# batra-mlp-lab/visdial

Measured on NVIDIA H100. Metric: QA-rounds/sec mn-att-ques-im-hist+disc train step, higher is better.
Workload: dtype f16 operands + f16 saved state for the option LSTM, tf32 operands elsewhere; fp32 accumulate, fp32 cell state / gradients / optimiser

## Files before the change

### visdial_b200/csrc/engine.cu

```cuda
#include "engine.h"
#include <string.h>
#include <math.h>
#include <cmath>

namespace vd {

Cfg parse_cfg(const vd_params* p) {
  VD_REQUIRE(p && p->encoder && p->decoder, VD_E_BADARG, "params / encoder / decoder is null");
  Cfg c;
  c.encoder = p->encoder; c.decoder = p->decoder;
  struct { const char* name; int enc; } known[] = {
      {"lf-ques", ENC_LF_QUES}, {"lf-ques-im-hist", ENC_LF_QIH}, {"hrea-ques-im-hist", ENC_HREA}, {"mn-att-ques-im-hist", ENC_MN_ATT},
      {"lf-ques-im", ENC_LF_QI}, {"lf-ques-hist", ENC_LF_QH}, {"hre-ques-hist", ENC_HRE_QH}, {"hre-ques-im-hist", ENC_HRE_QIH},
      {"mn-ques-hist", ENC_MN_QH}, {"mn-ques-im-hist", ENC_MN_QIH}, {"lf-att-ques-im-hist", ENC_LF_ATT}};
  c.enc = -1;
  for (auto& k : known)
    if (c.encoder == k.name) c.enc = k.enc;
  VD_REQUIRE(c.enc >= 0, VD_E_BADARG, "unknown encoder (one of the eleven names of encoders/*.lua)");
  if (c.decoder == "disc") c.dec = DEC_DISC;
  else if (c.decoder == "gen") c.dec = DEC_GEN;
  else VD_REQUIRE(false, VD_E_BADARG, "unknown decoder (disc | gen)");
  c.V = p->vocabSize; c.E = p->embedSize; c.H = p->rnnHiddenSize; c.L = p->numLayers; c.F = p->imgFeatureSize;
  c.S = p->imgSpatialSize; c.IE = p->imgEmbedSize; c.Cm = p->commonEmbeddingSize; c.hops = p->numAttentionLayers;
  c.R = p->maxQuesCount; c.K = p->numOptions; c.dropout = p->dropout; c.gpuid = p->gpuid;
// ... 53 lines not shown
    }
    add_linear(l, "san.out", c.H, c.H);
  };
  if (c.fam_lf && !c.san) {
    add_lstm(l, "ques.lstm1", c.E, c.H); add_lstm(l, "ques.lstm2", c.H, c.H);
    if (c.useHist) { add_lstm(l, "hist.lstm1", c.E, c.H); add_lstm(l, "hist.lstm2", c.H, c.H); }
    add_linear(l, "fusion", c.H, c.H + (c.useIm ? c.F : 0) + (c.useHist ? c.H : 0));
  } else if (c.fam_hre) {
    if (c.img_in_q) add_linear(l, "img.embed", c.IE, c.F);
    add_lstm(l, "hist.lstm1", c.E, c.H); add_lstm(l, "hist.lstm2", c.H, c.H);
    add_lstm(l, "ques.lstm1", c.E + (c.img_in_q ? c.IE : 0), c.H); add_lstm(l, "ques.lstm2", c.H, c.H);
    if (c.hre_att) { add_linear(l, "att.q", 1, c.H); add_linear(l, "att.h", 1, c.H); }
    add_lstm(l, "dialog.lstm", 2 * c.H, c.H);
  } else {
    add_lstm(l, "hist.lstm1", c.E, c.H); add_lstm(l, "hist.lstm2", c.H, c.H);
    add_lstm(l, "ques.lstm1", c.E, c.H); add_lstm(l, "ques.lstm2", c.H, c.H);
    if (c.fam_lf) add_linear(l, "fusion", c.H, 2 * c.H);
    if (c.mn_qi) add_linear(l, "mn.qi", c.H, c.H + c.F);
    if (c.fam_mn) { add_linear(l, "mn.fact", c.H, c.H); add_linear(l, "mn.query", c.H, c.H); }
    if (c.san) add_san();
  }
  if (c.dec == DEC_DISC) {
    add_lstm(l, "opt.lstm", c.E, c.H);
  } else {
    add_lstm(l, "dec.lstm1", c.E, c.H); add_lstm(l, "dec.lstm2", c.H, c.H);
    add_linear(l, "dec.out", c.V, c.H);
  }
  return l;
}

void* Arena::alloc(size_t bytes) {
  bytes = (bytes + 255) & ~(size_t)255;
  if (bytes == 0) bytes = 256;
  while (cur < chunks.size()) {
    Chunk& c = chunks[cur];
    if (c.used + bytes <= c.cap) { void* p = c.p + c.used; c.used += bytes; return p; }
    ++cur;
  }
  Chunk c; c.cap = std::max<size_t>(bytes, (size_t)256 << 20); c.used = bytes;
  VD_CUDA_CHECK(cudaMalloc((void**)&c.p, c.cap));
  chunks.push_back(c);
  cur = chunks.size() - 1;
  return c.p;
}
void Arena::reset() { for (auto& c : chunks) c.used = 0; cur = 0; }
void Arena::release() { for (auto& c : chunks) cudaFree(c.p); chunks.clear(); cur = 0; }
void Arena::rewind(const Mark& m) {
  for (size_t i = m.chunk; i < chunks.size(); ++i) chunks[i].used = i == m.chunk ? m.used : 0;
  cur = m.chunk;
}

void* GrowBuf::ensure(size_t bytes) {
  if (bytes > cap) {
    if (p) cudaFree(p);
    p = nullptr; cap = 0;
    VD_CUDA_CHECK(cudaMalloc(&p, bytes));
    cap = bytes;
  }
  return p;
}
void GrowBuf::release() { if (p) cudaFree(p); p = nullptr; cap = 0; }

Engine::Engine(const vd_params* p) {
  cfg = parse_cfg(p);
  lay = build_layout(cfg);
  nparams = lay.total;
  int ndev = 0;
  VD_CUDA_CHECK(cudaGetDeviceCount(&ndev));
  VD_REQUIRE(cfg.gpuid >= 0 && cfg.gpuid < ndev, VD_E_BADARG, "gpuid out of range");
  VD_CUDA_CHECK(cudaSetDevice(cfg.gpuid));
  cudaDeviceProp prop;
  VD_CUDA_CHECK(cudaGetDeviceProperties(&prop, cfg.gpuid));
  VD_REQUIRE(prop.major == 9 && prop.minor == 0, VD_E_CUDA, "visdial_b200 is built for sm_90a (H100) only");
  cx.sm_count = prop.multiProcessorCount;
  int prio_lo = 0, prio_hi = 0;
  VD_CUDA_CHECK(cudaDeviceGetStreamPriorityRange(&prio_lo, &prio_hi));
  VD_CUDA_CHECK(cudaStreamCreateWithPriority(&cx.stream, cudaStreamNonBlocking, prio_hi));
  main_stream = cx.stream;
  VD_CUDA_CHECK(cudaStreamCreateWithPriority(&side_stream, cudaStreamNonBlocking, prio_hi));
  main_chain.a = main_stream; side_chain.a = side_stream;
  for (cudaStream_t* s : {&main_chain.b, &side_chain.b, &main_chain.c, &side_chain.c})
    VD_CUDA_CHECK(cudaStreamCreateWithPriority(s, cudaStreamNonBlocking, prio_hi));
  VD_CUDA_CHECK(cudaStreamCreateWithPriority(&opt_stream, cudaStreamNonBlocking, prio_lo));
  VD_CUDA_CHECK(cudaEventCreateWithFlags(&ev_fork, cudaEventDisableTiming));
  VD_CUDA_CHECK(cudaEventCreateWithFlags(&ev_join, cudaEventDisableTiming));
  VD_CUDA_CHECK(cudaEventCreateWithFlags(&ev_opt_fork, cudaEventDisableTiming));
  VD_CUDA_CHECK(cudaEventCreateWithFlags(&ev_opt_done, cudaEventDisableTiming));
  size_t bytes = (size_t)nparams * sizeof(float);
  VD_CUDA_CHECK(cudaMalloc((void**)&W, bytes));
  VD_CUDA_CHECK(cudaMalloc((void**)&dW, bytes));
  VD_CUDA_CHECK(cudaMalloc((void**)&m, bytes));
  VD_CUDA_CHECK(cudaMalloc((void**)&v, bytes));
  VD_CUDA_CHECK(cudaMalloc((void**)&Wt, bytes));
  VD_CUDA_CHECK(cudaMemsetAsync(W, 0, bytes, cx.stream));
  VD_CUDA_CHECK(cudaMemsetAsync(dW, 0, bytes, cx.stream));
  VD_CUDA_CHECK(cudaMemsetAsync(m, 0, bytes, cx.stream));
  VD_CUDA_CHECK(cudaMemsetAsync(v, 0, bytes, cx.stream));
  VD_CUDA_CHECK(cudaMemsetAsync(Wt, 0, bytes, cx.stream));
  VD_CUDA_CHECK(cudaMalloc((void**)&scalars_dev, 64 * sizeof(float)));
  std::vector<int64_t> tab;
  for (auto& s : lay.segs) {
    if (s.init == VD_INIT_LSTM_W || s.init == VD_INIT_LINEAR_W) {
      tab.push_back(s.off); tab.push_back(s.rows); tab.push_back(s.cols);
      max2d = std::max(max2d, s.rows * s.cols);
    }
  }
  nseg2d = (int)tab.size() / 3;
  VD_CUDA_CHECK(cudaMalloc((void**)&segtab_dev, tab.size() * sizeof(int64_t)));
  VD_CUDA_CHECK(cudaMemcpyAsync(segtab_dev, tab.data(), tab.size() * sizeof(int64_t), cudaMemcpyHostToDevice, cx.stream));
  VD_CUDA_CHECK(cudaStreamSynchronize(cx.stream));
  VD_CUDA_CHECK(cudaEventCreate(&t0));
  VD_CUDA_CHECK(cudaEventCreate(&t1));
}

Engine::~Engine() {
  cudaSetDevice(cfg.gpuid);
  cudaStreamSynchronize(cx.stream);
  if (opt_stream) cudaStreamSynchronize(opt_stream);
  arena.release();
  for (auto& g : stage) g.release();
  for (auto& g : dense_buf) g.release();
  dialog_hist.release();
  for (auto& g : dialog_out) g.release();
  if (copy_stream) {
    cudaStreamSynchronize(copy_stream); cudaStreamDestroy(copy_stream);
    cudaEventDestroy(ev_img_ready); cudaEventDestroy(ev_copy_fork);
    for (auto ev : ev_img_free) cudaEventDestroy(ev);
  }
  for (auto& g : stage_img) g.release();
  cudaFree(W); cudaFree(dW); cudaFree(m); cudaFree(v); cudaFree(Wt); cudaFree(scalars_dev); cudaFree(segtab_dev);
  if (flush_buf) cudaFree(flush_buf);
  cx.collect();
  for (auto e : cx.free_events) cudaEventDestroy(e);
  if (t0) cudaEventDestroy(t0);
  if (t1) cudaEventDestroy(t1);
  if (ev_fork) cudaEventDestroy(ev_fork);
  if (ev_join) cudaEventDestroy(ev_join);
  if (side_stream) { cudaStreamSynchronize(side_stream); cudaStreamDestroy(side_stream); }
  for (cudaStream_t s : {main_chain.b, side_chain.b, main_chain.c, side_chain.c})
    if (s) { cudaStreamSynchronize(s); cudaStreamDestroy(s); }
  if (opt_stream) { cudaStreamSynchronize(opt_stream); cudaStreamDestroy(opt_stream); }
  if (ev_opt_fork) cudaEventDestroy(ev_opt_fork);
  if (ev_opt_done) cudaEventDestroy(ev_opt_done);
  for (auto e : ev_pool) cudaEventDestroy(e);
  cudaStreamDestroy(main_stream);
}

int Engine::seg(const char* name) const {
  int i = lay.find(name);
  VD_REQUIRE(i >= 0, VD_E_STATE, name);
  return i;
}

DropCfg Engine::dropcfg(float p) const {
  DropCfg d;
  d.seed_lo = (uint32_t)drop_seed; d.seed_hi = (uint32_t)(drop_seed >> 32); d.iter = (uint32_t)drop_iter;
  if (training == 1 && p > 0.f) {
    double t = (double)p * 4294967296.0;
    d.thresh = (uint32_t)std::min(t, 4294967295.0);
    d.scale = 1.f / (1.f - p);
  } else { d.thresh = 0; d.scale = 1.f; }
  return d;
}

void Engine::gemm_tn(int M, int N, int K, const float* A, int64_t lda, const int32_t* gather, const float* B, int64_t ldb,
                     float* C, int64_t ldc, float beta, const float* bias, int act) {
  LaunchCtx::Scope sc(&cx, "gemm", 2.0 * M * N * K, 4.0 * ((double)M * K + (double)N * K + (double)M * N));
  if (tcmode() && gemm_tn_tc(cx, M, N, K, A, lda, gather, B, ldb, C, ldc, beta, bias, act)) return;
  gemm_tn_simt(cx, M, N, K, A, lda, gather, B, ldb, C, ldc, beta, bias, act);
}
void Engine::gemm_atb(int M, int N, int64_t K, const float* A, int64_t lda, const int32_t* gather, const float* B,
                      int64_t ldb, float* C, int64_t ldc) {
  LaunchCtx::Scope sc(&cx, "gemm_wgrad", 2.0 * M * N * K, 4.0 * ((double)M * K + (double)N * K + (double)M * N));
  if (tcmode() && gemm_atb_tc(cx, M, N, K, A, lda, gather, B, ldb, C, ldc)) return;
  gemm_atb_simt(cx, M, N, K, A, lda, gather, B, ldb, C, ldc);
}

void Engine::linear_fwd(int wseg, const float* x, int64_t rows, float* y, int act) {
  const Seg& s = lay.segs[wseg];
  gemm_tn((int)rows, (int)s.rows, (int)s.cols, x, s.cols, nullptr, Wp(wseg), s.cols, y, s.rows, 0.f, Wp(wseg + 1), act);
}
void Engine::linear_bwd(int wseg, const float* x, const float* dy, int64_t rows, float* dx, float beta_dx) {
  const Seg& s = lay.segs[wseg];
  int out = (int)s.rows, in = (int)s.cols;
  gemm_atb(out, in, rows, dy, out, nullptr, x, in, dWp(wseg), in);
  colsum_add(cx, dWp(wseg + 1), dy, rows, out, out);
  if (dx) gemm_tn((int)rows, in, out, dy, out, nullptr, Wtp(wseg), out, dx, in, beta_dx, nullptr, 0);
}

void Engine::refresh_shadows() {
  VD_CUDA_CHECK(cudaMemsetAsync(W, 0, (size_t)cfg.E * sizeof(float), cx.stream));
  transpose_segments(cx, W, Wt, segtab_dev, nseg2d, max2d);
}

void Engine::stage_batch(const vd_batch* b) {
  VD_REQUIRE(b != nullptr, VD_E_BADARG, "batch is null");
  VD_REQUIRE(b->B > 0, VD_E_SHAPE, "batch B must be > 0");
  db = DevBatch();
  db.B = b->B; db.N = (int64_t)b->B * cfg.R;
  db.Tq = b->Tq; db.Th = b->Th; db.Ta = b->Ta; db.To = b->To;
  VD_REQUIRE(b->ques_fwd && b->Tq > 0, VD_E_SHAPE, "ques_fwd / Tq missing");
  if (cfg.useHist) VD_REQUIRE(b->hist && b->Th > 0, VD_E_SHAPE, "encoder uses history: hist / Th missing");
  if (cfg.useIm) VD_REQUIRE(b->img_feat, VD_E_SHAPE, "encoder uses the image: img_feat missing");
  int64_t img_elems = cfg.att ? (int64_t)b->B * cfg.S * cfg.S * cfg.F : (int64_t)b->B * cfg.F;
  struct Item { const void* src; size_t bytes; const void** dst; } items[9] = {
      {b->ques_fwd, (size_t)db.N * b->Tq * 4, (const void**)&db.ques},
      {cfg.useHist ? b->hist : nullptr, (size_t)db.N * b->Th * 4, (const void**)&db.hist},
      {cfg.useIm ? b->img_feat : nullptr, (size_t)img_elems * 4, (const void**)&db.img},
      {b->options, (size_t)db.N * cfg.K * b->To * 4, (const void**)&db.options},
      {b->answer_ind, (size_t)db.N * 4, (const void**)&db.answer_ind},
      {b->answer_in, (size_t)db.N * b->Ta * 4, (const void**)&db.answer_in},
      {b->answer_out, (size_t)db.N * b->Ta * 4, (const void**)&db.answer_out},
      {b->option_in, (size_t)db.N * cfg.K * b->To * 4, (const void**)&db.option_in},
      {b->option_out, (size_t)db.N * cfg.K * b->To * 4, (const void**)&db.option_out}};
  img_copy_pending = false;
  for (int i = 0; i < 9; ++i) {
    if (!items[i].src || items[i].bytes == 0) { *items[i].dst = nullptr; continue; }
    if (b->on_device) { *items[i].dst = items[i].src; continue; }
    if (i == 2 && items[i].bytes >= ((size_t)1 << 20)) {
      if (!copy_stream) {
        VD_CUDA_CHECK(cudaStreamCreateWithFlags(&copy_stream, cudaStreamNonBlocking));
        VD_CUDA_CHECK(cudaEventCreateWithFlags(&ev_img_ready, cudaEventDisableTiming));
        VD_CUDA_CHECK(cudaEventCreateWithFlags(&ev_copy_fork, cudaEventDisableTiming));
        for (int k = 0; k < 2; ++k) VD_CUDA_CHECK(cudaEventCreateWithFlags(&ev_img_free[k], cudaEventDisableTiming));
      }
      img_slot ^= 1;
// ... 232 lines not shown
    VD_CUDA_CHECK(cudaEventRecord(ex, s.c));
    VD_CUDA_CHECK(cudaStreamWaitEvent(s.b, ex, 0));
    cx.stream = s.b;
    lstm_forward_step(l2, t, true);
  }
  VD_CUDA_CHECK(cudaEventRecord(e0, s.b));
  VD_CUDA_CHECK(cudaStreamWaitEvent(s.a, e0, 0));
  cx.stream = s.a;
}

void Engine::lstm_backward_begin(LstmRun& r, const float* dh_all, const float* dh_last, const float* dc_last) {
  VD_REQUIRE(r.saved, VD_E_STATE, "lstm_backward needs a forward run in training mode");
  const int H = r.H, G = 4 * r.H;
  const int64_t R = r.R, TR = (int64_t)r.T * R;
  r.dc_carry = arena.get<float>(R * H);
  r.bw_dh_all = dh_all; r.bw_dh_last = dh_last;
  if (r.route.bwd == LstmPath::Opt16) {
    VD_REQUIRE(dh_last && !dh_all && !dc_last, VD_E_STATE, "fp16 BPTT takes its gradient from the last step only");
    r.da16 = arena.get<__half>(TR * G);
    r.scale2 = arena.get<float>(4);
    pick_grad_scale(cx, dh_last, R * H, reinterpret_cast<uint32_t*>(r.scale2 + 2), r.scale2);
    return;
  }
  r.da = arena.get<float>(TR * G);
  r.dh_rec = arena.get<float>(R * H);
  if (dc_last)
    VD_CUDA_CHECK(cudaMemcpyAsync(r.dc_carry, dc_last, (size_t)R * H * sizeof(float), cudaMemcpyDeviceToDevice, cx.stream));
  else
    VD_CUDA_CHECK(cudaMemsetAsync(r.dc_carry, 0, (size_t)R * H * sizeof(float), cx.stream));
}

void Engine::lstm_backward_step(LstmRun& r, int t) {
  const int H = r.H, G = 4 * r.H;
  const int64_t R = r.R, RH = R * H, RG = R * G;
  const bool last = t == r.T - 1;
  const float* cp = t > 0 ? r.c + (t - 1) * RH : r.c0;
  const int32_t* mk = r.mask ? r.mask + (int64_t)t * R : nullptr;
  if (r.route.bwd == LstmPath::Opt16) {
    const __half* g16 = r.gates16 + t * RG;
    __half* da16_t = r.da16 + t * RG;
    if (last) {
      LaunchCtx::Scope sc(&cx, "lstm_step_bwd_last", 0.0, R * (2.0 * G + 2.0 * G + 16.0 * H));
      lstm16_bwd_last(cx, R, H, g16, cp, r.c + t * RH, r.bw_dh_last, r.scale2, mk, r.dc_carry, da16_t);
    } else {
      LaunchCtx::Scope sc(&cx, "lstm_step_bwd", 2.0 * R * G * H, R * (3.0 * 2.0 * G + 16.0 * H));
      lstm16_step_bwd(cx, R, H, r.da16 + (t + 1) * RG, r.Whb16, g16, cp, r.c + t * RH, r.dc_carry, mk, da16_t);
    }
    return;
  }
  LstmBwdStep s;
  s.R = R; s.H = H; s.Wh = Wp(r.wseg) + (int64_t)r.D * G; s.dc_carry = r.dc_carry; s.dh_rec = r.dh_rec; s.mask = mk;
  s.da_next = last ? nullptr : r.da + (t + 1) * RG; s.dh_last = last ? r.bw_dh_last : nullptr;
  s.dh_ext = r.bw_dh_all ? r.bw_dh_all + t * RH : nullptr;
  s.gates = r.gates + t * RG; s.c_prev = cp; s.c_cur = r.c + t * RH; s.da = r.da + t * RG;
  const bool tc = r.route.bwd == LstmPath::Tc;
  LaunchCtx::Scope sc(&cx, (last && tc) ? "lstm_step_bwd_last" : (R >= 4096 ? "lstm_step_bwd" : "lstm_step_bwd_small"),
                      last ? 0.0 : 2.0 * R * G * H, 4.0 * R * (2.0 * G + 5.0 * H));
  if (tc) lstm_tc_bwd_step(s); else lstm_simt_bwd_step(s);
}

void Engine::lstm_backward_end(LstmRun& r, float* dx_out, float* dh0_out, float* dc0_out) {
  const int H = r.H, D = r.D, G = 4 * r.H;
  const int64_t R = r.R, TR = (int64_t)r.T * R;
  const float* Ws = Wp(r.wseg);
  float* dWs = dWp(r.wseg);
  const bool opt16 = r.route.bwd == LstmPath::Opt16;
  if (opt16) VD_REQUIRE(!dh0_out && !dc0_out && !dx_out && !r.h0, VD_E_STATE, "fp16 BPTT: no initial-state / input gradients");
  if (dh0_out) gemm_tn((int)R, H, G, r.da, G, nullptr, Ws + (int64_t)D * G, G, dh0_out, H, 0.f, nullptr, 0);
  if (dc0_out) VD_CUDA_CHECK(cudaMemcpyAsync(dc0_out, r.dc_carry, (size_t)R * H * sizeof(float), cudaMemcpyDeviceToDevice, cx.stream));
  const bool wgrad16 = opt16 || (r.route.bwd == LstmPath::Pair16 && TR - R >= 256);
  if (r.T > 1) {
    if (wgrad16) {
      LaunchCtx::Scope sc(&cx, "gemm_wgrad", 2.0 * H * G * (double)(TR - R), 2.0 * (double)(TR - R) * (H + G));
      const int budget = cx.sm_budget;
      cx.sm_budget = 0;
      gemm_atb16(cx, H, G, TR - R, r.h16, H, r.da16 + R * G, G, dWs + (int64_t)D * G, G, r.scale2 + 1);
      cx.sm_budget = budget;
    } else gemm_atb(H, G, TR - R, r.h, H, nullptr, r.da + R * G, G, dWs + (int64_t)D * G, G);
  }
  if (r.h0) gemm_atb(H, G, R, r.h0, H, nullptr, r.da, G, dWs + (int64_t)D * G, G);
  if (r.route.table_grad) {
    VD_REQUIRE(dx_out == nullptr, VD_E_STATE, "projected-space embedding gradient: caller must not ask for dx");
    const int V1 = cfg.V + 1;
    float* dP = arena.get<float>((int64_t)V1 * G);
    VD_CUDA_CHECK(cudaMemsetAsync(dP, 0, (size_t)V1 * G * sizeof(float), cx.stream));
    int32_t* scratch = arena.get<int32_t>(3 * (int64_t)V1);
    int32_t* perm = arena.get<int32_t>(TR);
    int32_t* stok = arena.get<int32_t>(TR);
    {
      LaunchCtx::Scope sc(&cx, "embed_grad_segsum", 0.0, (opt16 ? 2.0 : 4.0) * TR * G);
      group_rows_by_token(cx, r.gather, TR, V1, scratch, perm, stok);
      if (opt16) segsum_rows16(cx, r.da16, G, perm, stok, TR, dP, G, r.scale2 + 1);
      else segsum_rows(cx, r.da, G, perm, stok, TR, dP, G);
    }
    gemm_atb(D, G, V1, Wp(0), cfg.E, nullptr, dP, G, dWs, G);
    colsum_add(cx, dWp(r.wseg + 1), dP, V1, G, G);
    if (r.demb_out) gemm_tn(V1, D, G, dP, G, nullptr, Ws, G, r.demb_out, cfg.E, 0.f, nullptr, 0);
    else gemm_tn(V1, D, G, dP, G, nullptr, Ws, G, dWp(0), cfg.E, 1.f, nullptr, 0);
    return;
  }
  if (wgrad16 && r.x16) {
    LaunchCtx::Scope sc(&cx, "gemm_wgrad", 2.0 * D * G * (double)TR, 2.0 * (double)TR * (D + G));
    gemm_atb16(cx, D, G, TR, r.x16, D, r.da16, G, dWs, G, r.scale2 + 1);
  } else gemm_atb(D, G, TR, r.x ? r.x : Wp(0), r.x ? D : cfg.E, r.gather, r.da, G, dWs, G);
  colsum_add(cx, dWp(r.wseg + 1), r.da, TR, G, G);
  if (dx_out) gemm_tn((int)TR, D, G, r.da, G, nullptr, Ws, G, dx_out, D, 0.f, nullptr, 0);
}

void Engine::lstm_backward(LstmRun& r, const float* dh_all, const float* dh_last, const float* dc_last, float* dx_out,
                           float* dh0_out, float* dc0_out) {
  lstm_backward_begin(r, dh_all, dh_last, dc_last);
  for (int t = r.T - 1; t >= 0; --t) lstm_backward_step(r, t);
  lstm_backward_end(r, dx_out, dh0_out, dc0_out);
}

void Engine::lstm_pair_backward(LstmRun& l1, LstmRun& l2, const float* dh_last2, const float* dc_last2, const float* dh_last1,
                                const float* dc_last1, float* dx1_out, const PairStreams& s) {
  const int H = l2.H, G = 4 * l2.H;
  const int64_t R = l2.R;
  cx.stream = s.a;
  if (l1.route.bwd == LstmPath::Pair16) {
    const int T = l2.T;
    const int64_t TR = (int64_t)T * R;
    l1.da = arena.get<float>(TR * G); l2.da = arena.get<float>(TR * G);
    l1.da16 = arena.get<__half>(TR * G); l2.da16 = arena.get<__half>(TR * G);
    __half* Whb2 = arena.get<__half>((int64_t)H * G);
    __half* B1cat = arena.get<__half>((int64_t)H * 2 * G);
    cvt_f32_to_f16(cx, Whb2, G, Wp(l2.wseg) + (int64_t)l2.D * G, G, H, G);
    cvt_f32_to_f16(cx, B1cat, 2 * G, Wp(l2.wseg), G, H, G);
    cvt_f32_to_f16(cx, B1cat + G, 2 * G, Wp(l1.wseg) + (int64_t)l1.D * G, G, H, G);
    int* flags = arena.get<int>(enc_pair_bwd_flag_ints(T, R, H));
    float* dh1 = nullptr; float* dh2 = nullptr;
    if (enc_pair_gate_split(H)) { dh1 = arena.get<float>(TR * H); dh2 = arena.get<float>(TR * H); }
    l1.scale2 = l2.scale2 = arena.get<float>(2);
    {
      LaunchCtx::Scope sc2(&cx, "enc_pair_bwd", 2.0 * T * R * (double)H * 3.0 * G, 4.0 * T * R * (4.0 * G + 4.0 * H));
      enc_pair_backward(cx, T, R, H, B1cat, Whb2, l1.mask, l1.gates, l1.c, l2.gates, l2.c, dh_last1, dc_last1, dh_last2, dc_last2,
                        l1.da, l1.da16, l2.da, l2.da16, flags, dh1, dh2, l1.scale2);
    }
    lstm_backward_end(l2, nullptr, nullptr, nullptr);
    lstm_backward_end(l1, dx1_out, nullptr, nullptr);
    return;
  }
  float* dx2 = arena.get<float>((int64_t)l2.T * R * l2.D);
  if (!l1.route.wave_bwd) {
    lstm_backward(l2, nullptr, dh_last2, dc_last2, dx2, nullptr, nullptr);
    lstm_backward(l1, dx2, dh_last1, dc_last1, dx1_out, nullptr, nullptr);
    return;
  }
  const float* Wx2 = Wp(l2.wseg);
  cudaEvent_t e0 = pool_event(0);
  VD_CUDA_CHECK(cudaEventRecord(e0, s.a));
  VD_CUDA_CHECK(cudaStreamWaitEvent(s.b, e0, 0));
  cx.stream = s.b;
  lstm_backward_begin(l2, nullptr, dh_last2, dc_last2);
  cx.stream = s.a;
  lstm_backward_begin(l1, dx2, dh_last1, dc_last1);
  for (int t = l2.T - 1; t >= 0; --t) {
    cx.stream = s.b;
    lstm_backward_step(l2, t);
    cudaEvent_t e = pool_event(1 + t);
    VD_CUDA_CHECK(cudaEventRecord(e, s.b));
    VD_CUDA_CHECK(cudaStreamWaitEvent(s.c, e, 0));
    cx.stream = s.c;
    gemm_tn((int)R, l2.D, G, l2.da + (int64_t)t * R * G, G, nullptr, Wx2, G, dx2 + (int64_t)t * R * l2.D, l2.D, 0.f, nullptr, 0);
    cudaEvent_t ex = pool_event(1 + l2.T + t);
    VD_CUDA_CHECK(cudaEventRecord(ex, s.c));
    VD_CUDA_CHECK(cudaStreamWaitEvent(s.a, ex, 0));
    cx.stream = s.a;
    lstm_backward_step(l1, t);
  }
  cx.stream = s.b;
  lstm_backward_end(l2, nullptr, nullptr, nullptr);
  VD_CUDA_CHECK(cudaEventRecord(e0, s.b));
  cx.stream = s.a;
  lstm_backward_end(l1, dx1_out, nullptr, nullptr);
  VD_CUDA_CHECK(cudaStreamWaitEvent(s.a, e0, 0));
}

static LstmRun make_run(int T, int64_t R, int D, int H, int wseg, const float* x, const int32_t* gather, const int32_t* mask) {
  LstmRun r; r.T = T; r.R = R; r.D = D; r.H = H; r.wseg = wseg; r.x = x; r.gather = gather; r.mask = mask;
  return r;
}

void Engine::mn_block_fwd(const float* qin, const float* h3, float* out) {
  const int H = cfg.H, R = cfg.R, B = db.B;
  const int64_t N = db.N;
  const DropCfg d05 = dropcfg(0.5f);
  probs = arena.get<float>((int64_t)B * R * R);
// ... 276 lines not shown
      san_block_bwd(dEnc, du);
      mn_block_bwd(du, qh2, dqin, dh3);
    } else {
      mn_block_bwd(dEnc, encOut, dqin, dh3);
    }
    if (cfg.mn_qi) {
      tanh_bwd(cx, dpre, dqin, qi_proj, N * H);
      float* dqj = arena.get<float>(N * (H + cfg.F));
      linear_bwd(seg("mn.qi.weight"), qi_join, dpre, N, dqj, 0.f);
      copy_cols(cx, dq3, H, dqj, H + cfg.F, N, H);
    }
    if (cfg.san) reduce_segments(seg(cfg.mn_qi ? "mn.qi.weight" : "mn.fact.weight"), seg("san.out.weight") + 1, main_stream);
  }

  const bool embdrop = cfg.embdrop;
  if (cfg.useHist) {
    if (serial_pairs()) join_side(); else fork_side();
    const PairStreams& hs = serial_pairs() ? main_chain : side_chain;
    float* dx1 = arena.get<float>(N * db.Th * E);
    lstm_pair_backward(hist1, hist2, dh3, nullptr, nullptr, nullptr, dx1, hs);
    reduce_segments(seg("hist.lstm1.weight"), seg("hist.lstm2.weight") + 1, hs.a);
    embed_scatter_add(cx, dWp(0), dx1, E, ids_h, N * db.Th, E, embdrop ? d05 : dnone, SITE_HEMBED);
    back_to_main();
  }
  {
    int D1 = ques1.D;
    float* dx1 = arena.get<float>(N * db.Tq * D1);
    lstm_pair_backward(ques1, ques2, dq3, conn_dc_l2, conn_dh_l1, conn_dc_l1, dx1, main_chain);
    reduce_segments(seg("ques.lstm1.weight"), seg("ques.lstm2.weight") + 1, main_stream);
    embed_scatter_add(cx, dWp(0), dx1, D1, ids_q, N * db.Tq, E, embdrop ? d05 : dnone, SITE_QEMBED);
    if (cfg.img_in_q) {
      float* die = arena.get<float>(N * cfg.IE);
      masktime_bwd(cx, dx1, D1, E, ids_q, die, db.Tq, N, cfg.IE);
      linear_bwd(seg("img.embed.weight"), img_d, die, N, nullptr, 0.f);
    }
  }
  join_side();
  join_options_backward();
}

void Engine::fork_side() {
  if (!side_active) {
    VD_CUDA_CHECK(cudaEventRecord(ev_fork, main_stream));
    VD_CUDA_CHECK(cudaStreamWaitEvent(side_stream, ev_fork, 0));
    side_active = true;
  }
  cx.stream = side_stream;
}
void Engine::back_to_main() { cx.stream = main_stream; }
void Engine::join_side() {
  cx.stream = main_stream;
  if (side_active) {
    VD_CUDA_CHECK(cudaEventRecord(ev_join, side_stream));
    VD_CUDA_CHECK(cudaStreamWaitEvent(main_stream, ev_join, 0));
    side_active = false;
  }
}

void Engine::forward_connect() {
  if (cfg.dec != DEC_GEN) return;
  VD_REQUIRE(have_fwd, VD_E_STATE, "forward_connect before encoder_forward");
  gen_h0[0] = gen_h0[1] = gen_c0[0] = gen_c0[1] = nullptr;
  if (cfg.rnn_layers) {
    gen_h0[0] = ques1.h_last(); gen_c0[0] = ques1.c_last();
    gen_c0[1] = ques2.c_last();
  }
  gen_h0[1] = encOut;
}

void Engine::options_forward_async() {
  const int64_t Ro = (dense_round ? db.B : db.N) * cfg.K;
  cudaStream_t s = opt_overlap ? opt_stream : main_stream;
  if (opt_overlap) {
    VD_CUDA_CHECK(cudaEventRecord(ev_opt_fork, main_stream));
    VD_CUDA_CHECK(cudaStreamWaitEvent(opt_stream, ev_opt_fork, 0));
  }
  cudaStream_t prev = cx.stream;
  cx.stream = s;
  if (opt_overlap) cx.sm_budget = cx.sm_count - (math_mode == VD_MATH_F16 ? 0 : opt_reserve_sms);
  ids_o = arena.get<int32_t>(Ro * db.To);
  if (dense_round) transpose_ids_rounds(cx, db.options, dense_round, ids_o, db.B, cfg.R, cfg.K, db.To);
  else transpose_ids(cx, db.options, ids_o, Ro, db.To);
  opt = make_run(db.To, Ro, cfg.E, cfg.H, seg("opt.lstm.weight"), nullptr, ids_o, nullptr);
  lstm_forward(opt, save_acts);
  VD_CUDA_CHECK(cudaEventRecord(ev_opt_done, s));
  cx.stream = prev;
  cx.sm_budget = 0;
  opt_fwd_pending = true;
}

void Engine::join_options_backward() {
  if (!opt_bwd_pending) return;
  opt_bwd_pending = false;
  cudaStream_t prev = cx.stream;
  cx.stream = main_stream;
  VD_CUDA_CHECK(cudaStreamWaitEvent(main_stream, ev_opt_done, 0));
  if (opt_demb) add_inplace(cx, dWp(0), opt_demb, (int64_t)(cfg.V + 1) * cfg.E);
  opt_demb = nullptr;
  cx.stream = prev;
}

void Engine::decoder_forward() {
  VD_REQUIRE(have_fwd, VD_E_STATE, "decoder_forward before encoder_forward");
  const int E = cfg.E, H = cfg.H, K = cfg.K;
  const int64_t N = db.N;
  if (cfg.dec == DEC_DISC) {
    VD_REQUIRE(db.options && db.To > 0, VD_E_SHAPE, "disc decoder: options / To missing");
    if (!opt_fwd_pending) options_forward_async();
    VD_CUDA_CHECK(cudaStreamWaitEvent(main_stream, ev_opt_done, 0));
    opt_fwd_pending = false;
    cx.stream = main_stream;
    scores = arena.get<float>(N * K);
    disc_scores_fwd(cx, opt.h_last(), encOut, scores, N, K, H);
  } else {
    VD_REQUIRE(db.answer_in && db.Ta > 0, VD_E_SHAPE, "gen decoder: answer_in / Ta missing");
    forward_connect();
    ids_ai = arena.get<int32_t>(N * db.Ta);
    transpose_ids(cx, db.answer_in, ids_ai, N, db.Ta);
    float* xa = arena.get<float>(N * db.Ta * E);
    embed_rows(cx, xa, Wp(0), ids_ai, N * db.Ta, E, dropcfg(0.f), 0);
    dec1 = make_run(db.Ta, N, E, H, seg("dec.lstm1.weight"), xa, nullptr, ids_ai);
    dec1.h0 = gen_h0[0]; dec1.c0 = gen_c0[0];
    lstm_forward(dec1, true);
    dec2 = make_run(db.Ta, N, H, H, seg("dec.lstm2.weight"), dec1.h, nullptr, ids_ai);
    dec2.h0 = gen_h0[1]; dec2.c0 = gen_c0[1];
    lstm_forward(dec2, true);
    fused_vocab_fwd = false;
    const int64_t rows = N * db.Ta;
    const int wo = seg("dec.out.weight");
    if (!want_logp && tcmode() && db.answer_out) {
      ids_ao = arena.get<int32_t>(rows);
      transpose_ids(cx, db.answer_out, ids_ao, N, db.Ta);
      voc_nparts = vocab_lse_nparts(cfg.V);
      voc_pm = arena.get<float>(rows * voc_nparts); voc_ps = arena.get<float>(rows * voc_nparts);
      voc_tl = arena.get<float>(rows); voc_lse = arena.get<float>(rows);
      LaunchCtx::Scope sc(&cx, "vocab_lse", 2.0 * rows * cfg.V * H, 4.0 * (rows * (double)H + (double)cfg.V * H + 2.0 * rows * voc_nparts));
      fused_vocab_fwd = vocab_lse_tc(cx, (int)rows, cfg.V, H, dec2.h, H, Wp(wo), H, Wp(wo + 1), ids_ao, voc_pm, voc_ps, voc_tl);
    }
    if (!fused_vocab_fwd) {
      logp = arena.get<float>(rows * cfg.V);
      linear_fwd(wo, dec2.h, rows, logp, 0);
      logsoftmax_rows(cx, logp, ids_ai, rows, cfg.V);
    } else {
      logp = nullptr;
    }
  }
}

float Engine::criterion_forward() {
  const int64_t N = db.N;
  if (cfg.dec == DEC_DISC) {
    VD_REQUIRE(scores && db.answer_ind, VD_E_STATE, "criterion: decoder_forward / answer_ind missing");
    row_loss = arena.get<float>(N);
    xent_fwd(cx, scores, db.answer_ind, row_loss, N, cfg.K);
    reduce_sum(cx, row_loss, scalars_dev, N, 1.f / (float)N);
  } else {
    VD_REQUIRE((logp || fused_vocab_fwd) && db.answer_out, VD_E_STATE, "criterion: decoder_forward / answer_out missing");
    row_loss = arena.get<float>(N * db.Ta);
    if (fused_vocab_fwd) {
      vocab_lse_finish(cx, voc_pm, voc_ps, voc_nparts, voc_tl, ids_ao, ids_ai, voc_lse, row_loss, -1.f, 0, N * db.Ta);
    } else {
      ids_ao = arena.get<int32_t>(N * db.Ta);
      transpose_ids(cx, db.answer_out, ids_ao, N, db.Ta);
      nll_fwd(cx, logp, ids_ao, ids_ai, row_loss, N * db.Ta, cfg.V);
    }
    reduce_sum(cx, row_loss, scalars_dev, N * db.Ta, 1.f);
  }
// ... 597 lines not shown
```

### visdial_b200/csrc/engine.h

```cpp
#pragma once
#include <functional>
#include <string>
#include <vector>
#include "../../include/visdial_b200.h"
#include "kernels.cuh"

namespace vd {

enum EncKind { ENC_LF_QUES = 0, ENC_LF_QIH = 1, ENC_HREA = 2, ENC_MN_ATT = 3, ENC_LF_QI = 4, ENC_LF_QH = 5, ENC_HRE_QH = 6, ENC_HRE_QIH = 7,
               ENC_MN_QH = 8, ENC_MN_QIH = 9, ENC_LF_ATT = 10 };
enum DecKind { DEC_DISC = 0, DEC_GEN = 1 };

struct Cfg {
  std::string encoder, decoder;
  int enc = 0, dec = 0;
  int V = 0, E = 300, H = 512, L = 2, F = 4096, S = 14, IE = 300, Cm = 512, hops = 1, R = 10, K = 100;
  float dropout = 0.5f;
  int gpuid = 0;
  bool useIm = false, useHist = false, att = false;
  bool fam_lf = false, fam_hre = false, fam_mn = false;
  bool hre_att = false;
  bool san = false;
  bool img_in_q = false;
  bool img_drop = false;
  bool mn_qi = false;
  bool embdrop = false;
  bool rnn_layers = false;
};
Cfg parse_cfg(const vd_params* p);

struct Seg {
  std::string name;
  int64_t off = 0, rows = 0, cols = 0;
  int init = 0;
  int64_t fan_in = 0;
};
struct Layout {
  std::vector<Seg> segs;
  int64_t total = 0;
  int find(const std::string& name) const;
};
Layout build_layout(const Cfg& c);

struct Arena {
  struct Chunk { char* p; size_t cap; size_t used; };
  std::vector<Chunk> chunks;
  size_t cur = 0;
  void* alloc(size_t bytes);
  template <typename T> T* get(int64_t n) { return reinterpret_cast<T*>(alloc((size_t)n * sizeof(T))); }
  void reset();
  void release();
  struct Mark { size_t chunk, used; };
  Mark mark() const { return {cur, cur < chunks.size() ? chunks[cur].used : 0}; }
  void rewind(const Mark& m);
};

enum class LstmPath { Simt, Tc, Opt16, Pair16 };
struct LstmRoute {
  LstmPath fwd = LstmPath::Simt, bwd = LstmPath::Simt;
  bool table_grad = false;
  bool wave_fwd = false, wave_bwd = false;
};

struct LstmRun {
  int T = 0; int64_t R = 0; int D = 0, H = 0;
  int wseg = -1;
  const float* x = nullptr;
  const int32_t* gather = nullptr;
  const int32_t* mask = nullptr;
  const float* h0 = nullptr; const float* c0 = nullptr;
  float* h = nullptr; float* c = nullptr; float* gates = nullptr;
  bool saved = false;
  float* demb_out = nullptr;
  LstmRoute route;
  const float* ptable = nullptr;
  float* da = nullptr; float* dc_carry = nullptr; float* dh_rec = nullptr;
  const float* bw_dh_all = nullptr; const float* bw_dh_last = nullptr;
  __half *h16 = nullptr, *gates16 = nullptr, *da16 = nullptr, *P16 = nullptr, *Wh16 = nullptr, *Whb16 = nullptr;
  const __half* x16 = nullptr;
  float* h32_last = nullptr;
  float* scale2 = nullptr;
  const float* h_last() const { return route.fwd == LstmPath::Opt16 ? h32_last : h + (int64_t)(saved ? T - 1 : (T - 1) & 1) * R * H; }
  const float* c_last() const { return c + (int64_t)(saved ? T - 1 : (T - 1) & 1) * R * H; }
};

struct LstmFwdStep {
  int64_t R = 0, ldw = 0; int H = 0;
  const float *WhT = nullptr, *bias = nullptr, *h_prev = nullptr, *c_prev = nullptr, *ptable = nullptr;
  const int32_t *tok = nullptr, *mask = nullptr;
  float *gates = nullptr, *c_out = nullptr, *h_out = nullptr;
};
struct LstmBwdStep {
  int64_t R = 0; int H = 0;
  const float *Wh = nullptr, *da_next = nullptr, *dh_last = nullptr, *dh_ext = nullptr, *gates = nullptr, *c_prev = nullptr,
              *c_cur = nullptr;
  const int32_t* mask = nullptr;
  float *dc_carry = nullptr, *da = nullptr, *dh_rec = nullptr;
};

struct DevBatch {
  int B = 0, Tq = 0, Th = 0, Ta = 0, To = 0; int64_t N = 0;
  const int32_t* ques = nullptr; const int32_t* hist = nullptr; const float* img = nullptr;
  const int32_t* options = nullptr; const int32_t* answer_ind = nullptr;
  const int32_t* answer_in = nullptr; const int32_t* answer_out = nullptr;
  const int32_t* option_in = nullptr; const int32_t* option_out = nullptr;
};

struct GrowBuf {
  void* p = nullptr; size_t cap = 0;
  void* ensure(size_t bytes);
  void release();
};

struct Engine {
  Cfg cfg;
  Layout lay;
  LaunchCtx cx;
  int64_t nparams = 0;
  float *W = nullptr, *dW = nullptr, *m = nullptr, *v = nullptr, *Wt = nullptr;
  int64_t adam_t = 0;
  int64_t* segtab_dev = nullptr; int nseg2d = 0; int64_t max2d = 0;
  int training = 1;
  uint64_t drop_seed = 1234, drop_iter = 0;
  int math_mode = VD_MATH_TF32;
  bool tcmode() const { return math_mode != VD_MATH_FP32; }
  Arena arena;
  GrowBuf stage[9];
  GrowBuf stage_img[2];
  cudaStream_t copy_stream = nullptr;
  cudaEvent_t ev_img_ready = nullptr, ev_img_free[2] = {nullptr, nullptr}, ev_copy_fork = nullptr;
  int img_slot = 0;
  bool img_copy_pending = false, img_free_recorded[2] = {false, false};
  void wait_img();
  void release_img();
  DevBatch db;
  float* scalars_dev = nullptr;
  float* flush_buf = nullptr; int64_t flush_n = 0;
  cudaEvent_t t0 = nullptr, t1 = nullptr;
  cudaStream_t main_stream = nullptr, side_stream = nullptr;
  struct PairStreams { cudaStream_t a = nullptr, b = nullptr, c = nullptr; };
  PairStreams main_chain, side_chain;
  cudaEvent_t ev_fork = nullptr, ev_join = nullptr;
  bool side_active = false;
  void fork_side();
  void back_to_main();
  void join_side();

  void* nccl_comm = nullptr; int rank = 0, world = 1;

  bool have_fwd = false, save_acts = false;
  int32_t *ids_q = nullptr, *ids_h = nullptr, *ids_o = nullptr, *ids_ai = nullptr, *ids_ao = nullptr;
  float *xq = nullptr, *xh = nullptr;
  LstmRun ques1, ques2, hist1, hist2, dialog, opt, dec1, dec2;
  float *encOut = nullptr;
  float *join_d = nullptr; int joinK = 0;
  float *img_d = nullptr, *img_e = nullptr, *qi_in = nullptr, *sq = nullptr, *sh = nullptr, *probs = nullptr,
        *att = nullptr, *jt = nullptr, *dial_out = nullptr;
  float *hAtt = nullptr, *hAtt_d = nullptr, *hAttTr = nullptr, *sum1 = nullptr, *qh2 = nullptr, *t_img = nullptr,
        *img_tr = nullptr, *u_d = nullptr;
  std::vector<float*> img_common, ques_common, sc, pr, u_hop;
  float *scores = nullptr, *dscores = nullptr, *row_loss = nullptr, *logp = nullptr, *dlogits = nullptr,
        *lhood = nullptr;
  const float *gen_h0[2] = {nullptr, nullptr}, *gen_c0[2] = {nullptr, nullptr};
  float *gen_dh0[2] = {nullptr, nullptr}, *gen_dc0[2] = {nullptr, nullptr};
  float *dEncFromDec = nullptr;
  bool want_logp = true, fused_vocab_fwd = false;
  float *voc_pm = nullptr, *voc_ps = nullptr, *voc_tl = nullptr, *voc_lse = nullptr;
  int voc_nparts = 0;
  const float *conn_dh_l1 = nullptr, *conn_dc_l1 = nullptr, *conn_dc_l2 = nullptr;

  explicit Engine(const vd_params* p);
  ~Engine();

  const float* Wp(int seg) const { return W + lay.segs[seg].off; }
  const float* Wtp(int seg) const { return Wt + lay.segs[seg].off; }
  float* dWp(int seg) const { return dW + lay.segs[seg].off; }
  int seg(const char* name) const;
  DropCfg dropcfg(float p) const;
  void gemm_tn(int M, int N, int K, const float* A, int64_t lda, const int32_t* gather, const float* B, int64_t ldb,
               float* C, int64_t ldc, float beta, const float* bias, int act);
  void gemm_atb(int M, int N, int64_t K, const float* A, int64_t lda, const int32_t* gather, const float* B, int64_t ldb,
                float* C, int64_t ldc);
  void linear_fwd(int wseg, const float* x, int64_t rows, float* y, int act);
  void linear_bwd(int wseg, const float* x, const float* dy, int64_t rows, float* dx, float beta_dx);
  void refresh_shadows();
  void stage_batch(const vd_batch* b);
  LstmRoute route_lstm(int64_t R, int H, bool gathered, bool has_h0, const float* WhT, int64_t ldw, const float* Wh) const;
  LstmRoute route_lstm(const LstmRun& r) const {
    return route_lstm(r.R, r.H, r.gather != nullptr, r.h0 != nullptr, Wtp(r.wseg) + r.D, r.D + r.H,
                      Wp(r.wseg) + (int64_t)r.D * 4 * r.H);
  }
  void route_lstm_pair(LstmRun& l1, LstmRun& l2) const;
  void lstm_simt_fwd_step(const LstmFwdStep& s);
  int lstm_tc_fwd_step(const LstmFwdStep& s);
  void lstm_simt_bwd_step(const LstmBwdStep& s);
  int lstm_tc_bwd_step(const LstmBwdStep& s);
  void lstm_forward(LstmRun& r, bool save);
  void lstm_forward_begin(LstmRun& r, bool save, bool xproj_by_caller = false);
  void lstm_forward_step(LstmRun& r, int t, bool xproj_by_caller = false);
  void lstm_xproj(const LstmRun& r, int t0, int nt, float* gates);
  void lstm_backward_begin(LstmRun& r, const float* dh_all, const float* dh_last, const float* dc_last);
  void lstm_backward_step(LstmRun& r, int t);
  void lstm_backward_end(LstmRun& r, float* dx_out, float* dh0_out, float* dc0_out);
  void lstm_pair_forward(LstmRun& l1, LstmRun& l2, const PairStreams& s);
  void lstm_pair_backward(LstmRun& l1, LstmRun& l2, const float* dh_last2, const float* dc_last2, const float* dh_last1,
                          const float* dc_last1, float* dx1_out, const PairStreams& s);
  bool serial_pairs() const { return cfg.useHist && hist1.route.fwd == LstmPath::Pair16; }
  cudaStream_t opt_stream = nullptr;
  cudaEvent_t ev_opt_fork = nullptr, ev_opt_done = nullptr;
  bool opt_overlap = true, opt_fwd_pending = false, opt_bwd_pending = false;
  int opt_reserve_sms = 16;
  float* opt_demb = nullptr;
  void options_forward_async();
  void options_backward(const float* dfeat);
  void join_options_backward();
  const int32_t* dense_round = nullptr;
  GrowBuf dense_buf[2];
  float forward_backward_dense(const vd_batch* b, const int32_t* round_host, const float* relevance_host);
  std::vector<cudaEvent_t> ev_pool;
  cudaEvent_t pool_event(size_t i);
  void lstm_backward(LstmRun& r, const float* dh_all, const float* dh_last, const float* dc_last, float* dx_out,
                     float* dh0_out, float* dc0_out);

  void encoder_forward(const vd_batch* b);
  void encoder_backward(const float* dEnc);
  float *qi_join = nullptr, *qi_proj = nullptr;
  const float* mn_query_in = nullptr;
  void mn_block_fwd(const float* qin, const float* h3, float* out);
  void mn_block_bwd(const float* dout, const float* out, float* dqin, float* dh3);
  void san_block_fwd(const float* u0);
  void san_block_bwd(const float* dEnc, float* du0);
  void forward_connect();
  void decoder_forward();
  float criterion_forward();
  void criterion_backward();
  void decoder_backward();
  const float* backward_connect();
  void retrieve(const vd_batch* b, int use_gt, int32_t* ranks_host);
  void gen_option_lhood();
  LstmRun gstep1, gstep2;
  float* gstep_logp = nullptr;
  void gen_decoder_step(int64_t rows, const int32_t* tokens_host, const float* const* h_prev, const float* const* c_prev);
  void gen_decoder_step_logits(int64_t rows, const int32_t* tok, const float* const* h_prev, const float* const* c_prev);
  void gen_beam_search(int k, int L, int start_token, int end_token, int32_t* answer_host, int32_t* length_host, double* score_host);
  struct BeamResult { int32_t* ans; int32_t* len; double* score; };
  BeamResult beam_search_rows(int64_t n, int64_t stride, int64_t off, int k, int L, int start_token, int end_token);
  void gen_decoder_step_lstm(int64_t rows, const int32_t* tok, const float* const* h_prev, const float* const* c_prev);
  void gen_sample(int L, int start_token, float temperature, uint64_t seed, int64_t row_offset, int32_t* answer_host,
                  float* logp_host);
  void check_sample_args(int L, int start_token, float temperature, int64_t row_offset) const;
  struct SampleResult { int32_t* ans; float* logp; };
  SampleResult sample_rows(int64_t n, int64_t stride, int64_t off, int L, int start_token, float temperature, uint64_t seed,
                           int64_t row_offset);
  struct DialogAnswers {
    const int32_t* tokens; int64_t ld;
    const int32_t* len;
    int max_tokens;
    int end_token;
  };
  GrowBuf dialog_hist, dialog_out[4];
  void gen_dialog(const vd_batch* b, int W, int max_ans_len, const std::function<DialogAnswers(int)>& search, int32_t* hist_host);
  void gen_dialog_beam_search(const vd_batch* b, int k, int L, int start_token, int end_token, int W, int max_ans_len,
                              int32_t* answer_host, int32_t* length_host, double* score_host, int32_t* hist_host);
  void gen_dialog_sample(const vd_batch* b, int L, int start_token, int end_token, float temperature, uint64_t seed,
                         int64_t row_offset, int W, int max_ans_len, int32_t* answer_host, float* logp_host, int32_t* hist_host);
  GrowBuf pool_tok, pool_emb, pool_scratch;
  int64_t pool_m = 0; int pool_w = 0; bool pool_valid = false;
  void answer_pool_encode(const int32_t* tokens_host, int64_t m, int w);
  void pool_topk(const float* Q, int64_t ldq, int64_t rows, const float* E, int64_t m, int H, int k, float* topv, int32_t* topi);
  void check_pool(int k) const;
  void answer_pool_retrieve(const vd_batch* b, int k, int32_t* index_host, float* score_host);
  void answer_pool_dialog(const vd_batch* b, int k, int W, int max_ans_len, int32_t* index_host, float* score_host,
                          int32_t* hist_host);
  void clamp_adam_step(float lr);
  void allreduce_grads();
  cudaStream_t comm_stream = nullptr;
  cudaEvent_t ev_comm_dep = nullptr, ev_comm_done = nullptr;
  std::vector<char> seg_reduced;
  bool ar_overlap = true, ar_armed = false, comm_pending = false;
  void reduce_range(int64_t off, int64_t count, cudaStream_t producer, cudaEvent_t producer_event);
  void reduce_segments(int first, int last, cudaStream_t producer, cudaEvent_t producer_event = nullptr);
  void reduce_remaining();
  void arm_grad_sync();
};

}
```

Baseline: 16140.

## Precompute option-LSTM token grouping on a side stream during forward

Moves the token sort/grouping and the zeroing of the projected-embedding gradient buffer out of the option LSTM backward. They now run during the option forward on a separate low-priority stream that joins before the options-done event. The backward segment-sum reuses the stored permutation, and the subsequent weight-gradient GEMMs run with the SM budget lifted. The cost is an extra stream and event pair, plus arena buffers that must stay alive from forward to backward.

```diff
diff --git a/visdial_b200/csrc/engine.cu b/visdial_b200/csrc/engine.cu
--- a/visdial_b200/csrc/engine.cu
+++ b/visdial_b200/csrc/engine.cu
@@ -159,10 +159,13 @@
   for (cudaStream_t* s : {&main_chain.b, &side_chain.b, &main_chain.c, &side_chain.c})
     VD_CUDA_CHECK(cudaStreamCreateWithPriority(s, cudaStreamNonBlocking, prio_hi));
   VD_CUDA_CHECK(cudaStreamCreateWithPriority(&opt_stream, cudaStreamNonBlocking, prio_lo));
+  VD_CUDA_CHECK(cudaStreamCreateWithPriority(&opt_sort_stream, cudaStreamNonBlocking, prio_lo));
   VD_CUDA_CHECK(cudaEventCreateWithFlags(&ev_fork, cudaEventDisableTiming));
   VD_CUDA_CHECK(cudaEventCreateWithFlags(&ev_join, cudaEventDisableTiming));
   VD_CUDA_CHECK(cudaEventCreateWithFlags(&ev_opt_fork, cudaEventDisableTiming));
   VD_CUDA_CHECK(cudaEventCreateWithFlags(&ev_opt_done, cudaEventDisableTiming));
+  VD_CUDA_CHECK(cudaEventCreateWithFlags(&ev_sort_fork, cudaEventDisableTiming));
+  VD_CUDA_CHECK(cudaEventCreateWithFlags(&ev_sort_done, cudaEventDisableTiming));
   size_t bytes = (size_t)nparams * sizeof(float);
   VD_CUDA_CHECK(cudaMalloc((void**)&W, bytes));
   VD_CUDA_CHECK(cudaMalloc((void**)&dW, bytes));
@@ -194,6 +197,7 @@
   cudaSetDevice(cfg.gpuid);
   cudaStreamSynchronize(cx.stream);
   if (opt_stream) cudaStreamSynchronize(opt_stream);
+  if (opt_sort_stream) cudaStreamSynchronize(opt_sort_stream);
   arena.release();
   for (auto& g : stage) g.release();
   for (auto& g : dense_buf) g.release();
@@ -219,6 +223,9 @@
   if (opt_stream) { cudaStreamSynchronize(opt_stream); cudaStreamDestroy(opt_stream); }
   if (ev_opt_fork) cudaEventDestroy(ev_opt_fork);
   if (ev_opt_done) cudaEventDestroy(ev_opt_done);
+  if (opt_sort_stream) { cudaStreamSynchronize(opt_sort_stream); cudaStreamDestroy(opt_sort_stream); }
+  if (ev_sort_fork) cudaEventDestroy(ev_sort_fork);
+  if (ev_sort_done) cudaEventDestroy(ev_sort_done);
   for (auto e : ev_pool) cudaEventDestroy(e);
   cudaStreamDestroy(main_stream);
 }
@@ -617,21 +624,19 @@
   if (r.route.table_grad) {
     VD_REQUIRE(dx_out == nullptr, VD_E_STATE, "projected-space embedding gradient: caller must not ask for dx");
     const int V1 = cfg.V + 1;
-    float* dP = arena.get<float>((int64_t)V1 * G);
-    VD_CUDA_CHECK(cudaMemsetAsync(dP, 0, (size_t)V1 * G * sizeof(float), cx.stream));
-    int32_t* scratch = arena.get<int32_t>(3 * (int64_t)V1);
-    int32_t* perm = arena.get<int32_t>(TR);
-    int32_t* stok = arena.get<int32_t>(TR);
+    if (!r.tok_perm) group_tokens(r);
     {
       LaunchCtx::Scope sc(&cx, "embed_grad_segsum", 0.0, (opt16 ? 2.0 : 4.0) * TR * G);
-      group_rows_by_token(cx, r.gather, TR, V1, scratch, perm, stok);
-      if (opt16) segsum_rows16(cx, r.da16, G, perm, stok, TR, dP, G, r.scale2 + 1);
-      else segsum_rows(cx, r.da, G, perm, stok, TR, dP, G);
-    }
-    gemm_atb(D, G, V1, Wp(0), cfg.E, nullptr, dP, G, dWs, G);
-    colsum_add(cx, dWp(r.wseg + 1), dP, V1, G, G);
-    if (r.demb_out) gemm_tn(V1, D, G, dP, G, nullptr, Ws, G, r.demb_out, cfg.E, 0.f, nullptr, 0);
-    else gemm_tn(V1, D, G, dP, G, nullptr, Ws, G, dWp(0), cfg.E, 1.f, nullptr, 0);
+      if (opt16) segsum_rows16(cx, r.da16, G, r.tok_perm, r.tok_sorted, TR, r.dP, G, r.scale2 + 1);
+      else segsum_rows(cx, r.da, G, r.tok_perm, r.tok_sorted, TR, r.dP, G);
+    }
+    const int budget = cx.sm_budget;
+    cx.sm_budget = 0;
+    gemm_atb(D, G, V1, Wp(0), cfg.E, nullptr, r.dP, G, dWs, G);
+    colsum_add(cx, dWp(r.wseg + 1), r.dP, V1, G, G);
+    if (r.demb_out) gemm_tn(V1, D, G, r.dP, G, nullptr, Ws, G, r.demb_out, cfg.E, 0.f, nullptr, 0);
+    else gemm_tn(V1, D, G, r.dP, G, nullptr, Ws, G, dWp(0), cfg.E, 1.f, nullptr, 0);
+    cx.sm_budget = budget;
     return;
   }
   if (wgrad16 && r.x16) {
@@ -640,6 +645,17 @@
   } else gemm_atb(D, G, TR, r.x ? r.x : Wp(0), r.x ? D : cfg.E, r.gather, r.da, G, dWs, G);
   colsum_add(cx, dWp(r.wseg + 1), r.da, TR, G, G);
   if (dx_out) gemm_tn((int)TR, D, G, r.da, G, nullptr, Ws, G, dx_out, D, 0.f, nullptr, 0);
+}
+
+void Engine::group_tokens(LstmRun& r) {
+  const int V1 = cfg.V + 1, G = 4 * r.H;
+  const int64_t TR = (int64_t)r.T * r.R;
+  int32_t* scratch = arena.get<int32_t>(3 * (int64_t)V1);
+  r.tok_perm = arena.get<int32_t>(TR);
+  r.tok_sorted = arena.get<int32_t>(TR);
+  r.dP = arena.get<float>((int64_t)V1 * G);
+  group_rows_by_token(cx, r.gather, TR, V1, scratch, r.tok_perm, r.tok_sorted);
+  VD_CUDA_CHECK(cudaMemsetAsync(r.dP, 0, (size_t)V1 * G * sizeof(float), cx.stream));
 }
 
 void Engine::lstm_backward(LstmRun& r, const float* dh_all, const float* dh_last, const float* dc_last, float* dx_out,
@@ -1082,7 +1098,20 @@
   if (dense_round) transpose_ids_rounds(cx, db.options, dense_round, ids_o, db.B, cfg.R, cfg.K, db.To);
   else transpose_ids(cx, db.options, ids_o, Ro, db.To);
   opt = make_run(db.To, Ro, cfg.E, cfg.H, seg("opt.lstm.weight"), nullptr, ids_o, nullptr);
+  if (opt_overlap) VD_CUDA_CHECK(cudaEventRecord(ev_sort_fork, s));
   lstm_forward(opt, save_acts);
+  if (save_acts && opt.route.table_grad) {
+    if (opt_overlap) {
+      VD_CUDA_CHECK(cudaStreamWaitEvent(opt_sort_stream, ev_sort_fork, 0));
+      cx.stream = opt_sort_stream;
+    }
+    group_tokens(opt);
+    if (opt_overlap) {
+      VD_CUDA_CHECK(cudaEventRecord(ev_sort_done, opt_sort_stream));
+      VD_CUDA_CHECK(cudaStreamWaitEvent(s, ev_sort_done, 0));
+      cx.stream = s;
+    }
+  }
   VD_CUDA_CHECK(cudaEventRecord(ev_opt_done, s));
   cx.stream = prev;
   cx.sm_budget = 0;
diff --git a/visdial_b200/csrc/engine.h b/visdial_b200/csrc/engine.h
--- a/visdial_b200/csrc/engine.h
+++ b/visdial_b200/csrc/engine.h
@@ -80,6 +80,8 @@
   const __half* x16 = nullptr;
   float* h32_last = nullptr;
   float* scale2 = nullptr;
+  int32_t *tok_perm = nullptr, *tok_sorted = nullptr;
+  float* dP = nullptr;
   const float* h_last() const { return route.fwd == LstmPath::Opt16 ? h32_last : h + (int64_t)(saved ? T - 1 : (T - 1) & 1) * R * H; }
   const float* c_last() const { return c + (int64_t)(saved ? T - 1 : (T - 1) & 1) * R * H; }
 };
@@ -202,12 +204,13 @@
   void lstm_backward_begin(LstmRun& r, const float* dh_all, const float* dh_last, const float* dc_last);
   void lstm_backward_step(LstmRun& r, int t);
   void lstm_backward_end(LstmRun& r, float* dx_out, float* dh0_out, float* dc0_out);
+  void group_tokens(LstmRun& r);
   void lstm_pair_forward(LstmRun& l1, LstmRun& l2, const PairStreams& s);
   void lstm_pair_backward(LstmRun& l1, LstmRun& l2, const float* dh_last2, const float* dc_last2, const float* dh_last1,
                           const float* dc_last1, float* dx1_out, const PairStreams& s);
   bool serial_pairs() const { return cfg.useHist && hist1.route.fwd == LstmPath::Pair16; }
-  cudaStream_t opt_stream = nullptr;
-  cudaEvent_t ev_opt_fork = nullptr, ev_opt_done = nullptr;
+  cudaStream_t opt_stream = nullptr, opt_sort_stream = nullptr;
+  cudaEvent_t ev_opt_fork = nullptr, ev_opt_done = nullptr, ev_sort_fork = nullptr, ev_sort_done = nullptr;
   bool opt_overlap = true, opt_fwd_pending = false, opt_bwd_pending = false;
   int opt_reserve_sms = 16;
   float* opt_demb = nullptr;
```

Result: no change. 16180, median of 6 (+0.2%).
